# JiayuLi-997/IntEL-SIGIR2023

Hardware: AMD Instinct MI355X
Metric: train sessions/sec, IntEL fwd+IntBPRloss+bwd+Adam, synthetic Tmall-shape list=50 K=3, item / score tower 128 / 64 wide (higher is better)
Workload: dtype f32; 1 GPU; tmall: 1000000 items, list=50, K=3 rankers, I=30 intents, H=20, emb 64/64/64/64 (id/meta/score/ctx), BERT4Rec, 1 heads x 1 tied layers, f32, IntBPRloss loss, cal_diversity=0, uniform item ids, 8 resident batches; global_batch=4096, per_gpu_batch=4096, parallelism=dp1, table_adam=dense sweep over the whole table every step

## Files before the change

### intel_sigir2023_amd/csrc/attn_p3.hip

```cpp
#include "kernels.h"
#include "planes.h"
#include <stdlib.h>

namespace {

#define AP_QB 64
#define AP_KB 32
#define LOG2E_F 1.4426950408889634f
#ifndef AP_DKV_DUAL
#define AP_DKV_DUAL 0
#endif
#ifndef AP_DKV_PRE
#define AP_DKV_PRE 0
#endif
#ifndef AP_DKV_OCC
#define AP_DKV_OCC 3
#endif
#define LN2_F 0.6931471805599453f

typedef short ap_s16x4 __attribute__((ext_vector_type(4)));
typedef short ap_s16x8 __attribute__((ext_vector_type(8)));

template <int DKT>
struct P3Tile {
  static constexpr int RB = DKT * 32;
  static constexpr int NCH = DKT * 2;
  static constexpr int PLANE = AP_KB * RB;
  static constexpr int BYTES = 3 * PLANE;
  __device__ __forceinline__ static int swz(int row) {
    if (DKT == 8) return ((row & 3) << 1) | ((row >> 3) & 1) | ((((row >> 2) ^ (row >> 3)) & 1) << 3);
    const int u = (row >> 1) & 7;
    return ((u & 1) << 1) | ((u >> 2) & 1) | ((((u >> 1) ^ (u >> 2)) & 1) << 2);
  }
  __device__ __forceinline__ static int off(int row, int ch) { return RB * row + 16 * (ch ^ swz(row)); }
};

__device__ __forceinline__ void split8(const f32x4& a, const f32x4& b, bf16x8& h, bf16x8& m, bf16x8& l) {
#pragma unroll
  for (int i = 0; i < 4; ++i) {
    __bf16 hh, mm, ll;
    planes::split1(a[i], hh, mm, ll);
    h[i] = hh; m[i] = mm; l[i] = ll;
    planes::split1(b[i], hh, mm, ll);
    h[4 + i] = hh; m[4 + i] = mm; l[4 + i] = ll;
  }
}

template <int DKT>
struct P3Stage {
  static constexpr int NCH = DKT * 2, NCK = DKT / 4;
  f32x4 v[NCK][2];
  __device__ __forceinline__ void load(const float* __restrict__ base, int ldg, int coff, int r0, int nrow, int tid) {
#pragma unroll
    for (int n = 0; n < NCK; ++n) {
      const int i = tid + n * 256, r = i / NCH, ch = i - r * NCH, row = r0 + r;
      v[n][0] = v[n][1] = f32x4{0.f, 0.f, 0.f, 0.f};
      if (row < nrow) {
        const float* p = base + (size_t)row * ldg + coff + 8 * ch;
        v[n][0] = *reinterpret_cast<const f32x4*>(p);
        v[n][1] = *reinterpret_cast<const f32x4*>(p + 4);
      }
    }
  }
  __device__ __forceinline__ void store(unsigned char* tile, int tid) const {
    using TL = P3Tile<DKT>;
#pragma unroll
    for (int n = 0; n < NCK; ++n) {
      const int i = tid + n * 256, r = i / NCH, ch = i - r * NCH;
      bf16x8 h, m, l;
#if AP_ABLATE & 2
      for (int e = 0; e < 4; ++e) { h[e] = (__bf16)v[n][0][e]; h[4 + e] = (__bf16)v[n][1][e]; }
      m = h; l = h;
#else
      split8(v[n][0], v[n][1], h, m, l);
#endif
      unsigned char* d = tile + TL::off(r, ch);
      *reinterpret_cast<bf16x8*>(d) = h;
      *reinterpret_cast<bf16x8*>(d + TL::PLANE) = m;
      *reinterpret_cast<bf16x8*>(d + 2 * TL::PLANE) = l;
    }
  }
};

struct Frag3 { bf16x8 h, m, l; };
#define AP_MFMA(a, b, c) __builtin_amdgcn_mfma_f32_16x16x32_bf16(a, b, c, 0, 0, 0)
#ifndef AP_ABLATE
#define AP_ABLATE 0
#endif
__device__ __forceinline__ f32x4 ap_mma3(const bf16x8& ah, const bf16x8& am, const bf16x8& al, const bf16x8& bh, const bf16x8& bm, const bf16x8& bl, f32x4 c) {
#if AP_ABLATE & 1
  return AP_MFMA(ah, bh, c);
#else
  return planes::mma<3>(ah, am, al, bh, bm, bl, c);
#endif
}
__device__ __forceinline__ void mma3x2(const Frag3& a1, const Frag3& b1, f32x4& c1, const Frag3& a2, const Frag3& b2, f32x4& c2) {
#if AP_ABLATE & 1
  c1 = AP_MFMA(a1.h, b1.h, c1); c2 = AP_MFMA(a2.h, b2.h, c2);
  return;
#endif
  c1 = AP_MFMA(a1.m, b1.m, c1); c2 = AP_MFMA(a2.m, b2.m, c2);
  c1 = AP_MFMA(a1.h, b1.l, c1); c2 = AP_MFMA(a2.h, b2.l, c2);
  c1 = AP_MFMA(a1.l, b1.h, c1); c2 = AP_MFMA(a2.l, b2.h, c2);
  c1 = AP_MFMA(a1.h, b1.m, c1); c2 = AP_MFMA(a2.h, b2.m, c2);
  c1 = AP_MFMA(a1.m, b1.h, c1); c2 = AP_MFMA(a2.m, b2.h, c2);
  c1 = AP_MFMA(a1.h, b1.h, c1); c2 = AP_MFMA(a2.h, b2.h, c2);
}

template <int DKT>
__device__ __forceinline__ void own_row_planes(const float* __restrict__ rowp, bool ok, int g, Frag3 (&f)[DKT / 2]) {
#pragma unroll
  for (int c = 0; c < DKT / 2; ++c) {
    f32x4 a = f32x4{0.f, 0.f, 0.f, 0.f}, b = a;
    if (ok) {
      a = *reinterpret_cast<const f32x4*>(rowp + 32 * c + 8 * g);
      b = *reinterpret_cast<const f32x4*>(rowp + 32 * c + 8 * g + 4);
    }
    split8(a, b, f[c].h, f[c].m, f[c].l);
  }
}

template <int DKT>
__device__ __forceinline__ Frag3 row_frag(const unsigned char* tile, int roff, int t, int c) {
  using TL = P3Tile<DKT>;
  const unsigned char* p = tile + (roff ^ (64 * c)) + t * 16 * TL::RB;
  return Frag3{*reinterpret_cast<const bf16x8*>(p), *reinterpret_cast<const bf16x8*>(p + TL::PLANE), *reinterpret_cast<const bf16x8*>(p + 2 * TL::PLANE)};
}
template <int DKT, bool PRE = true>
__device__ __forceinline__ void row_mma2(const unsigned char* tile1, int t1, const Frag3 (&b1)[DKT / 2], f32x4& acc1, const unsigned char* tile2, int t2,
                                         const Frag3 (&b2)[DKT / 2], f32x4& acc2, int roff) {
  Frag3 a1 = row_frag<DKT>(tile1, roff, t1, 0), a2 = row_frag<DKT>(tile2, roff, t2, 0);
#pragma unroll
  for (int c = 0; c < DKT / 2; ++c) {
    Frag3 n1 = a1, n2 = a2;
    if (PRE && c + 1 < DKT / 2) {
      n1 = row_frag<DKT>(tile1, roff, t1, c + 1);
      n2 = row_frag<DKT>(tile2, roff, t2, c + 1);
    }
    mma3x2(a1, b1[c], acc1, a2, b2[c], acc2);
    if (!PRE && c + 1 < DKT / 2) {
      n1 = row_frag<DKT>(tile1, roff, t1, c + 1);
      n2 = row_frag<DKT>(tile2, roff, t2, c + 1);
    }
    a1 = n1; a2 = n2;
  }
}

__device__ __forceinline__ bf16x8 tr_frag(const unsigned char* plane, int off_lo, int off_hi) {
  const ap_s16x4 lo = __builtin_amdgcn_ds_read_tr16_b64_v4i16((__attribute__((address_space(3))) ap_s16x4*)(plane + off_lo));
  const ap_s16x4 hi = __builtin_amdgcn_ds_read_tr16_b64_v4i16((__attribute__((address_space(3))) ap_s16x4*)(plane + off_hi));
  return __builtin_bit_cast(bf16x8, __builtin_shufflevector(lo, hi, 0, 1, 2, 3, 4, 5, 6, 7));
}
template <int DKT>
__device__ __forceinline__ Frag3 tr_frag3(const unsigned char* tile, int tlo, int thi, int dt) {
  using TL = P3Tile<DKT>;
  const int lo = tlo ^ (32 * dt), hi = thi ^ (32 * dt);
  return Frag3{tr_frag(tile, lo, hi), tr_frag(tile + TL::PLANE, lo, hi), tr_frag(tile + 2 * TL::PLANE, lo, hi)};
}
template <int DKT, bool PRE = true>
__device__ __forceinline__ void tr_mma2(f32x4 (&acc1)[DKT], const unsigned char* tile1, const Frag3& b1, f32x4 (&acc2)[DKT], const unsigned char* tile2,
                                        const Frag3& b2, int tlo, int thi) {
  Frag3 a1 = tr_frag3<DKT>(tile1, tlo, thi, 0), a2 = tr_frag3<DKT>(tile2, tlo, thi, 0);
#pragma unroll
  for (int dt = 0; dt < DKT; ++dt) {
    Frag3 n1 = a1, n2 = a2;
    if (PRE && dt + 1 < DKT) {
      n1 = tr_frag3<DKT>(tile1, tlo, thi, dt + 1);
      n2 = tr_frag3<DKT>(tile2, tlo, thi, dt + 1);
    }
    mma3x2(a1, b1, acc1[dt], a2, b2, acc2[dt]);
    if (!PRE && dt + 1 < DKT) {
      n1 = tr_frag3<DKT>(tile1, tlo, thi, dt + 1);
      n2 = tr_frag3<DKT>(tile2, tlo, thi, dt + 1);
    }
    a1 = n1; a2 = n2;
  }
}
template <int DKT>
__device__ __forceinline__ f32x4 row_mma1(const unsigned char* tile, int t, const Frag3 (&b)[DKT / 2], f32x4 acc, int roff) {
#pragma unroll
  for (int c = 0; c < DKT / 2; ++c) {
    const Frag3 a = row_frag<DKT>(tile, roff, t, c);
    acc = ap_mma3(a.h, a.m, a.l, b[c].h, b[c].m, b[c].l, acc);
  }
  return acc;
}
template <int DKT>
__device__ __forceinline__ void tr_mma1(f32x4 (&acc)[DKT], const unsigned char* tile, const Frag3& b, int tlo, int thi) {
#pragma unroll
  for (int dt = 0; dt < DKT; ++dt) {
    const Frag3 a = tr_frag3<DKT>(tile, tlo, thi, dt);
    acc[dt] = ap_mma3(a.h, a.m, a.l, b.h, b.m, b.l, acc[dt]);
  }
}
template <int DKT>
__device__ __forceinline__ void tr_mma(f32x4 (&acc)[DKT], const unsigned char* tile, const Frag3& b, int tlo, int thi) {
  Frag3 a1 = tr_frag3<DKT>(tile, tlo, thi, 0), a2 = tr_frag3<DKT>(tile, tlo, thi, 1);
#pragma unroll
  for (int dt = 0; dt < DKT; dt += 2) {
    Frag3 n1 = a1, n2 = a2;
    if (dt + 2 < DKT) {
      n1 = tr_frag3<DKT>(tile, tlo, thi, dt + 2);
      n2 = tr_frag3<DKT>(tile, tlo, thi, dt + 3);
    }
    mma3x2(a1, b, acc[dt], a2, b, acc[dt + 1]);
    a1 = n1; a2 = n2;
  }
}
template <int DKT>
__device__ __forceinline__ void tr_addr(int lane, int& tlo, int& thi) {
  using TL = P3Tile<DKT>;
  const int p = lane & 15, g = lane >> 4, q = p >> 2, pp = p & 3;
  tlo = TL::off(4 * g + q, pp >> 1) + 8 * (pp & 1);
  thi = TL::off(16 + 4 * g + q, pp >> 1) + 8 * (pp & 1);
}

template <int DKT>
__device__ __forceinline__ void dim_store(float* __restrict__ rowp, const f32x4 (&acc)[DKT], int g, float mul) {
#pragma unroll
  for (int dt = 0; dt < DKT; ++dt) *reinterpret_cast<f32x4*>(rowp + 16 * dt + 4 * g) = acc[dt] * mul;
}

struct ApBlock { int bh, y; };
__device__ __forceinline__ ApBlock ap_block(int nbh, int ny) {
  const int id = blockIdx.x;
  if ((nbh & 7) == 0) {
    const int slot = id >> 3, g = slot / ny;
    return ApBlock{g * 8 + (id & 7), slot - g * ny};
  }
  const int bh = id / ny;
  return ApBlock{bh, id - bh * ny};
}

template <int DKT>
__global__ __launch_bounds__(256, DKT == 8 ? 2 : 3) void attn_fwd_p3_kernel(const float* __restrict__ qkv, int T, int d, int heads,
                                                                            const int* __restrict__ key_len, float scale, float* __restrict__ out,
                                                                            float* __restrict__ lse, const int* __restrict__ row_off) {
  using TL = P3Tile<DKT>;
  extern __shared__ __attribute__((aligned(16))) unsigned char smem_p3[];
  unsigned char* Ks = smem_p3;
  unsigned char* Vs = smem_p3 + TL::BYTES;
  const int tid = threadIdx.x, lane = tid & 63, wave = tid >> 6, p = lane & 15, g = lane >> 4;
  const int ny = (T + AP_QB - 1) / AP_QB;
  const ApBlock blk = ap_block((int)gridDim.x / ny, ny);
  const int b = blk.bh / heads, h = blk.bh - b * heads;
  const int dk = d / heads, ldg = 3 * d;
  const int nkeys = key_len ? min(key_len[b], T) : T;
  const int nrow = row_off ? nkeys : T;
  const size_t row0 = row_off ? (size_t)row_off[b] : (size_t)b * T;
  if (blk.y * AP_QB >= nrow) return;
  const float* base = qkv + row0 * ldg;
  const int q = blk.y * AP_QB + wave * 16 + p;
  Frag3 qf[DKT / 2];
  own_row_planes<DKT>(base + (size_t)q * ldg + h * dk, q < nrow, g, qf);
  f32x4 oT[DKT];
#pragma unroll
  for (int i = 0; i < DKT; ++i) oT[i] = f32x4{0.f, 0.f, 0.f, 0.f};
  float m_run = -INFINITY, l_run = 0.f;
  const int roff = TL::off(p, g);
  int tlo, thi;
  tr_addr<DKT>(lane, tlo, thi);
  const float scale2 = scale * LOG2E_F;

  P3Stage<DKT> kreg, vreg;
  kreg.load(base, ldg, d + h * dk, 0, nrow, tid);
  vreg.load(base, ldg, 2 * d + h * dk, 0, nrow, tid);
  for (int kb = 0; kb < nkeys; kb += AP_KB) {
    __syncthreads();
    kreg.store(Ks, tid);
    vreg.store(Vs, tid);
    __syncthreads();
    if (kb + AP_KB < nkeys) {
      kreg.load(base, ldg, d + h * dk, kb + AP_KB, nrow, tid);
      vreg.load(base, ldg, 2 * d + h * dk, kb + AP_KB, nrow, tid);
    }
// ... 140 lines not shown
  }
}

template <int DKT>
__global__ __launch_bounds__(256, 4) void attn_bwd_dq_ds_p3_kernel(const float* __restrict__ qkv, const float* __restrict__ dS, int ldS, int T, int d,
                                                                   int heads, const int* __restrict__ key_len, float* __restrict__ dqkv,
                                                                   const int* __restrict__ row_off) {
  extern __shared__ __attribute__((aligned(16))) unsigned char smem_p3[];
  unsigned char* Ks = smem_p3;
  const int tid = threadIdx.x, lane = tid & 63, wave = tid >> 6, p = lane & 15, g = lane >> 4;
  const int ny = (T + AP_QB - 1) / AP_QB;
  const ApBlock blk = ap_block((int)gridDim.x / ny, ny);
  const int b = blk.bh / heads, h = blk.bh - b * heads;
  const int dk = d / heads, ldg = 3 * d;
  const int nkeys = key_len ? min(key_len[b], T) : T;
  const int nrow = row_off ? nkeys : T;
  const size_t row0 = row_off ? (size_t)row_off[b] : (size_t)b * T;
  if (blk.y * AP_QB >= nrow) return;
  const float* base = qkv + row0 * ldg;
  const int q = blk.y * AP_QB + wave * 16 + p;
  const bool qok = q < nrow;
  const float* dSq = dS + ((size_t)blk.bh * T + (qok ? q : 0)) * ldS;
  f32x4 dqT[DKT];
#pragma unroll
  for (int i = 0; i < DKT; ++i) dqT[i] = f32x4{0.f, 0.f, 0.f, 0.f};
  int tlo, thi;
  tr_addr<DKT>(lane, tlo, thi);
  P3Stage<DKT> kreg;
  kreg.load(base, ldg, d + h * dk, 0, nrow, tid);
  for (int kb = 0; kb < nkeys; kb += AP_KB) {
    __syncthreads();
    kreg.store(Ks, tid);
    __syncthreads();
    if (kb + AP_KB < nkeys) kreg.load(base, ldg, d + h * dk, kb + AP_KB, nrow, tid);
    if (blk.y * AP_QB + wave * 16 >= nrow) continue;
    f32x4 dsT[2];
#pragma unroll
    for (int kt = 0; kt < 2; ++kt) {
      const int key0 = kb + kt * 16 + 4 * g;
      dsT[kt] = f32x4{0.f, 0.f, 0.f, 0.f};
      if (qok && key0 < ldS && key0 < nkeys) dsT[kt] = *reinterpret_cast<const f32x4*>(dSq + key0);
#pragma unroll
      for (int r = 0; r < 4; ++r) dsT[kt][r] = key0 + r < nkeys ? dsT[kt][r] : 0.f;
    }
    Frag3 df;
    split8(dsT[0], dsT[1], df.h, df.m, df.l);
    tr_mma<DKT>(dqT, Ks, df, tlo, thi);
  }
  if (qok) dim_store<DKT>(dqkv + (row0 + q) * ldg + h * dk, dqT, g, 1.f);
}

}

bool attn_p3_supported(int T, int dk) {
  static const int on = [] { const char* e = getenv("INTEL_ATTN_P3"); return (e && e[0] == '0') ? 0 : 1; }();
  return on && gemm_planes() == 3 && T > 64 && (dk == 64 || dk == 128);
}

#define AP_DISPATCH(DKT_RT, CALL) \
  if ((DKT_RT) == 4) { constexpr int DKT = 4; CALL; } else { constexpr int DKT = 8; CALL; }

int launch_attn_p3_fwd(const float* qkv, int B, int T, int d, int heads, const int* key_len, float* out, float* lse, hipStream_t st, const int* row_off) {
  const int dk = d / heads, dkt = dk / 16;
  INTEL_CHECK_ARG(dk == 64 || dk == 128, "attention (bf16-plane kernels): head dim %d", dk);
  const float scale = 1.0f / sqrtf((float)dk);
  dim3 grid(B * heads * cdiv(T, AP_QB));
  AP_DISPATCH(dkt, {
    size_t smem = (size_t)2 * P3Tile<DKT>::BYTES;
    allow_lds(attn_fwd_p3_kernel<DKT>, smem);
    LAUNCH_S(B * heads, T, dk, 4.0 * B * T * (double)T * d, 16.0 * B * T * (double)d, attn_fwd_p3_kernel<DKT>, grid, dim3(256), smem, st, qkv, T, d, heads, key_len, scale, out, lse, row_off);
  });
  INTEL_CHECK_LAUNCH();
  return 0;
}

int launch_attn_p3_bwd(const float* qkv, const float* dout, const float* lse, const float* dsum, int B, int T, int d, int heads, const int* key_len,
                       float* dqkv, float* dS, int ldS, hipStream_t st, const int* row_off) {
  const int dk = d / heads, dkt = dk / 16;
  INTEL_CHECK_ARG(dk == 64 || dk == 128, "attention (bf16-plane kernels): head dim %d", dk);
  const float scale = 1.0f / sqrtf((float)dk);
  dim3 grid(B * heads * cdiv(T, AP_QB));
  AP_DISPATCH(dkt, {
    size_t smem = (size_t)2 * P3Tile<DKT>::BYTES + 2 * AP_KB * sizeof(float);
    allow_lds(attn_bwd_dkv_p3_kernel<DKT>, smem);
    LAUNCH_S(B * heads, T, dk, 8.0 * B * T * (double)T * d, 24.0 * B * T * (double)d, attn_bwd_dkv_p3_kernel<DKT>, grid, dim3(256), smem, st, qkv, dout, lse, dsum, T, d, heads,
             key_len, scale, dqkv, dS, ldS, row_off);
  });
  INTEL_CHECK_LAUNCH();
  AP_DISPATCH(dkt, {
    size_t smem = (size_t)P3Tile<DKT>::BYTES;
    allow_lds(attn_bwd_dq_ds_p3_kernel<DKT>, smem);
    LAUNCH_S(B * heads, T, dk, 2.0 * B * T * (double)T * d, 8.0 * B * T * (double)d + 4.0 * B * heads * (double)T * T, attn_bwd_dq_ds_p3_kernel<DKT>, grid, dim3(256), smem, st, qkv, dS,
             ldS, T, d, heads, key_len, dqkv, row_off);
  });
  INTEL_CHECK_LAUNCH();
  return 0;
}
```

### intel_sigir2023_amd/csrc/attn_seq.hip

```cpp
#include <stdio.h>
#include <stdlib.h>
#include "kernels.h"

namespace {

__device__ __forceinline__ int perm16(int r) { return (r & ~15) | ((r & 3) << 2) | ((r >> 2) & 3); }
__device__ __forceinline__ float gmax16(float v) {
  v = fmaxf(v, __shfl_xor(v, 16));
  return fmaxf(v, __shfl_xor(v, 32));
}
__device__ __forceinline__ float gsum16(float v) {
  v += __shfl_xor(v, 16);
  return v + __shfl_xor(v, 32);
}

typedef short s16x4 __attribute__((ext_vector_type(4)));
typedef __bf16 bf16x4s __attribute__((ext_vector_type(4)));
template <bool BF>
__device__ __forceinline__ f32x4 mma4(const f32x4& a, const f32x4& b, f32x4 c) {
  if (BF) {
    const bf16x4s ab = bf16x4s{(__bf16)a[0], (__bf16)a[1], (__bf16)a[2], (__bf16)a[3]};
    const bf16x4s bb = bf16x4s{(__bf16)b[0], (__bf16)b[1], (__bf16)b[2], (__bf16)b[3]};
    return __builtin_amdgcn_mfma_f32_16x16x16bf16_1k(__builtin_bit_cast(s16x4, ab), __builtin_bit_cast(s16x4, bb), c, 0, 0, 0);
  }
#pragma unroll
  for (int s = 0; s < 4; ++s) c = mfma16(a[s], b[s], c);
  return c;
}

template <bool H>
__device__ __forceinline__ f32x4 ldx4(const float* __restrict__ base, size_t off) {
  if (H) {
    const bf16x4s v = *reinterpret_cast<const bf16x4s*>(reinterpret_cast<const __bf16*>(base) + off);
    return f32x4{(float)v[0], (float)v[1], (float)v[2], (float)v[3]};
  }
  return *reinterpret_cast<const f32x4*>(base + off);
}
template <bool H>
__device__ __forceinline__ void stx4(float* __restrict__ base, size_t off, const f32x4& v) {
  if (H) *reinterpret_cast<bf16x4s*>(reinterpret_cast<__bf16*>(base) + off) = bf16x4s{(__bf16)v[0], (__bf16)v[1], (__bf16)v[2], (__bf16)v[3]};
  else *reinterpret_cast<f32x4*>(base + off) = v;
}

template <int DKT, int NT>
struct SeqP {
  static constexpr int DK = DKT * 16;
  static constexpr int PW = 4 / NT;
  static constexpr int TP = NT * 16;
  static constexpr int ROWS = PW * TP;
  static constexpr int CPR = DKT * 4;
  static constexpr int BUF = ROWS * DK;
  static constexpr int IPW = ROWS * CPR / 256;
};

template <int DKT, int NT, bool PERM>
// ... 226 lines not shown
};

template <int DKT, int NT, bool PERM>
__device__ __forceinline__ bool seq_src(int i, int bh0, int BH, int T, int heads, int& rl, int& c4, size_t& grow, int& hcol,
                                        const int* __restrict__ row_off = nullptr, const int* __restrict__ key_len = nullptr) {
  using C = SeqCfg<DKT, NT>;
  rl = i / C::C4;
  c4 = i - rl * C::C4;
  const int sl = rl / C::TP, r = rl - sl * C::TP;
  const int rho = PERM ? perm16(r) : r;
  const int bh = bh0 + sl;
  int b = bh, h = 0;
  if (heads > 1) { b = bh / heads; h = bh - b * heads; }
  hcol = h * C::DK + c4 * 4;
  if (row_off) {
    if (bh >= BH) { grow = 0; return false; }
    grow = (size_t)row_off[b] + rho;
    return rho < min(key_len[b], T);
  }
  grow = (size_t)b * T + rho;
  return bh < BH && rho < T;
}

template <int DKT, int NT, bool PERM, bool TWO>
__device__ __forceinline__ void stage_seq2(float* dst0, const float* __restrict__ src0, int ld0, int coff0, float* dst1,
                                           const float* __restrict__ src1, int ld1, int coff1, int bh0, int BH, int T,
                                           int heads, int tid) {
  using C = SeqCfg<DKT, NT>;
  f32x4 v0[C::ITERS], v1[C::ITERS];
#pragma unroll
  for (int it = 0; it < C::ITERS; ++it) {
    int rl, c4, hcol;
    size_t grow;
    const bool ok = seq_src<DKT, NT, PERM>(tid + it * 256, bh0, BH, T, heads, rl, c4, grow, hcol);
    const size_t gr = ok ? grow : 0;
    const int hc = ok ? hcol : 0;
    const f32x4 zero = f32x4{0.f, 0.f, 0.f, 0.f};
    const f32x4 t0 = *reinterpret_cast<const f32x4*>(src0 + gr * ld0 + coff0 + hc);
    v0[it] = ok ? t0 : zero;
    if (TWO) {
      const f32x4 t1 = *reinterpret_cast<const f32x4*>(src1 + gr * ld1 + coff1 + hc);
      v1[it] = ok ? t1 : zero;
    }
  }
#pragma unroll
  for (int it = 0; it < C::ITERS; ++it) {
    const int i = tid + it * 256;
    const int rl = i / C::C4, c4 = i - rl * C::C4;
    *reinterpret_cast<f32x4*>(dst0 + rl * C::LD + c4 * 4) = v0[it];
    if (TWO) *reinterpret_cast<f32x4*>(dst1 + rl * C::LD + c4 * 4) = v1[it];
  }
}

template <int DKT, int NT, int LS, bool BF = false, bool H16 = false>
__global__ __launch_bounds__(256, 2) void attn_seq_bwd_fused_kernel(const float* __restrict__ qkv, const float* __restrict__ out,
                                                              const float* __restrict__ dout, const float* __restrict__ lse,
                                                              int BH, int T, int d, int heads, const int* __restrict__ key_len,
                                                              const int* __restrict__ row_off, float c2, float scale,
                                                              float* __restrict__ dqkv) {
  using C = SeqCfg<DKT, NT>;
  constexpr int LD = C::LD, DK = C::DK, DQ = DKT / 4, TP = C::TP, NSTEPS = (NT - 1) * 4 + LS;
  extern __shared__ __attribute__((aligned(16))) float smem[];
  float* Qs = smem;
  float* Os = smem + C::ROWS * LD;
  float* Ls = smem + C::ROWS * LD + C::OSZ;
  float* Ds = Ls + C::ROWS;
  const int tid = threadIdx.x, lane = tid & 63, wave = tid >> 6, j = lane >> 4, p = lane & 15;
  const int bh0 = blockIdx.x * C::PW, ldg = 3 * d;
  const int slot = wave / NT, tile = wave - slot * NT, bh = bh0 + slot;
  const bool live = slot < C::PW && bh < BH;
  int b = live ? bh : 0, h = 0;
  if (heads > 1) { b = (live ? bh : 0) / heads; h = (live ? bh : 0) - b * heads; }
  const int key = tile * 16 + p;
  const size_t base = row_off ? (size_t)row_off[b] : (size_t)b * T;
  const int tb = row_off ? min(key_len[b], T) : T;
  const bool kok = live && key < tb;
  f32x4 kf[DKT], vf[DKT];
#pragma unroll
  for (int g = 0; g < DKT; ++g) {
    const int col = g * 16 + 4 * j;
    const bool ok = kok && col < DK;
    const size_t off = ok ? (base + key) * ldg + d + h * DK + col : 0;
    const f32x4 tk = ldx4<H16>(qkv, off), tv = ldx4<H16>(qkv, off + (ok ? d : 0));
    kf[g] = ok ? tk : f32x4{0.f, 0.f, 0.f, 0.f};
    vf[g] = ok ? tv : f32x4{0.f, 0.f, 0.f, 0.f};
  }
  {
    f32x4 vq[C::ITERS], vo[C::ITERS];
#pragma unroll
    for (int it = 0; it < C::ITERS; ++it) {
      int rl, c4, hcol;
      size_t grow;
      const bool ok = seq_src<DKT, NT, true>(tid + it * 256, bh0, BH, T, heads, rl, c4, grow, hcol, row_off, key_len);
      const size_t gr = ok ? grow : 0;
      const int hc = ok ? hcol : 0;
      const f32x4 zero = f32x4{0.f, 0.f, 0.f, 0.f};
      const f32x4 tq = ldx4<H16>(qkv, gr * ldg + hc);
      const f32x4 to = ldx4<H16>(dout, gr * d + hc);
      vq[it] = ok ? tq : zero;
      vo[it] = ok ? to : zero;
    }
#pragma unroll
    for (int it = 0; it < C::ITERS; ++it) {
      const int i = tid + it * 256;
      const int rl = i / C::C4, c4 = i - rl * C::C4;
      *reinterpret_cast<f32x4*>(Qs + rl * LD + c4 * 4) = vq[it];
      *reinterpret_cast<f32x4*>(Os + rl * LD + c4 * 4) = vo[it];
    }
    if (tid < C::ROWS) {
      const int sl = tid / TP, r = tid - sl * TP, rho = perm16(r), bb = bh0 + sl;
      const int tbb = (row_off && bb < BH) ? min(key_len[heads > 1 ? bb / heads : bb], T) : T;
      Ls[tid] = (bb < BH && rho < tbb) ? -1.44269504088896340736f * lse[(size_t)bb * T + rho] : -INFINITY;
// ... 210 lines not shown
bool attn_seq_supported(int T, int dk) {
  static const int off = [] { const char* e = getenv("INTEL_ATTN_SEQ"); return (e && e[0] == '0') ? 1 : 0; }();
  return !off && T >= 1 && T <= 64 && (dk == 64 || dk == 128);
}

int launch_attn_seq_fwd(const float* qkv, int B, int T, int d, int heads, const int* key_len, float* out, float* lse,
                        hipStream_t st, const int* row_off) {
  INTEL_CHECK_ARG(!row_off || key_len, "attn_seq: packed rows need the session lengths");
  const int dk = d / heads, dkt = dk / 16, BH = B * heads;
  const int nt = cdiv(T, 16), ls = cdiv(T - (nt - 1) * 16, 4);
  const float scale = 1.0f / sqrtf((float)dk);
  SEQ_DISPATCH3(dkt, nt, ls, {
    using C = SeqP<DKT, NT>;
    const size_t smem = (size_t)4 * C::BUF * sizeof(float);
    const int per_cu = (int)((size_t)160 * 1024 / smem);
    const int grid = min(cdiv(BH, C::PW), num_cus() * (per_cu < 1 ? 1 : per_cu));
    if (gemm_planes() == 1) {
      allow_lds((attn_seq_fwd_kernel<DKT, NT, LS, true>), smem);
      LAUNCH_S(BH, T, dk, 4.0 * B * T * (double)T * d, 16.0 * B * T * (double)d, (attn_seq_fwd_kernel<DKT, NT, LS, true>), dim3(grid), dim3(256), smem, st, qkv, BH, T, d, heads, key_len, row_off, scale * 1.44269504088896340736f, scale, out, lse);
    } else {
      allow_lds((attn_seq_fwd_kernel<DKT, NT, LS>), smem);
      LAUNCH_S(BH, T, dk, 4.0 * B * T * (double)T * d, 16.0 * B * T * (double)d, (attn_seq_fwd_kernel<DKT, NT, LS>), dim3(grid), dim3(256), smem, st, qkv, BH, T, d, heads, key_len, row_off, scale * 1.44269504088896340736f, scale, out, lse);
    }
  });
  INTEL_CHECK_LAUNCH();
  return 0;
}

size_t attn_seq_bwd_scratch_floats(int B, int T, int heads) {
  const size_t tp = (size_t)cdiv(T, 16) * 16;
  return (size_t)B * heads * tp * tp;
}

bool attn_seq_packed_supported(int T, int dk) {
  return attn_seq_supported(T, dk);
}

bool attn_seq_h16_supported(int T, int dk) { return attn_seq_packed_supported(T, dk) && gemm_planes() == 1; }

int launch_attn_seq_bwd(const float* qkv, const float* out, const float* dout, const float* lse, int B, int T, int d,
                        int heads, const int* key_len, float* dqkv, float* dS, hipStream_t st, const int* row_off, int h16) {
  INTEL_CHECK_ARG(!h16 || attn_seq_h16_supported(T, d / heads), "attn_seq: bf16-stored q/k/v need the fused backward in bf16 mode");
  INTEL_CHECK_ARG(!row_off || (key_len && attn_seq_packed_supported(T, d / heads)), "attn_seq: packed rows need the fused backward and the session lengths");
  const int dk = d / heads, dkt = dk / 16, BH = B * heads;
  const int nt = cdiv(T, 16), ls = cdiv(T - (nt - 1) * 16, 4);
  const float scale = 1.0f / sqrtf((float)dk);
  {
    SEQ_DISPATCH3(dkt, nt, ls, {
      using C = SeqCfg<DKT, NT>;
      const size_t smem = (size_t)(C::ROWS * C::LD + C::OSZ + (1 + NT) * C::ROWS) * sizeof(float);
      if (h16) {
        allow_lds((attn_seq_bwd_fused_kernel<DKT, NT, LS, true, true>), smem);
        LAUNCH_S(BH, T, dk, 10.0 * B * T * (double)T * d, 16.0 * B * T * (double)d, (attn_seq_bwd_fused_kernel<DKT, NT, LS, true, true>), dim3(cdiv(BH, C::PW)), dim3(256), smem, st, qkv, out, dout, lse, BH, T, d, heads, key_len, row_off, scale * 1.44269504088896340736f, scale, dqkv);
      } else if (gemm_planes() == 1) {
        allow_lds((attn_seq_bwd_fused_kernel<DKT, NT, LS, true>), smem);
        LAUNCH_S(BH, T, dk, 10.0 * B * T * (double)T * d, 24.0 * B * T * (double)d, (attn_seq_bwd_fused_kernel<DKT, NT, LS, true>), dim3(cdiv(BH, C::PW)), dim3(256), smem, st, qkv, out, dout, lse, BH, T, d, heads, key_len, row_off, scale * 1.44269504088896340736f, scale, dqkv);
      } else {
        allow_lds((attn_seq_bwd_fused_kernel<DKT, NT, LS>), smem);
        LAUNCH_S(BH, T, dk, 10.0 * B * T * (double)T * d, 24.0 * B * T * (double)d, (attn_seq_bwd_fused_kernel<DKT, NT, LS>), dim3(cdiv(BH, C::PW)), dim3(256), smem, st, qkv, out, dout, lse, BH, T, d, heads, key_len, row_off, scale * 1.44269504088896340736f, scale, dqkv);
      }
    });
    INTEL_CHECK_LAUNCH();
    return 0;
  }
}
```

### intel_sigir2023_amd/csrc/kernels.h

```cpp
#pragma once
#include "common.h"

static inline size_t packed_floats(int Kd, int Nd) { return (size_t)rup(Kd, 16) * rup(Nd, 16); }
int launch_pack_b(const float* W, int ldw, int Kd, int Nd, int trans, float* P, int nt_off, hipStream_t st,
                  int g_off = 0, int KG_total = 0);

void pack_batch_begin();
int pack_batch_end(hipStream_t st);

struct GemmEpilogue {
  const float* bias = nullptr;
  int relu = 0;
  const float* mask = nullptr;
  int ldmask = 0;
  const float* res = nullptr;
  int ldres = 0;
  const float* gamma = nullptr;
  const float* beta = nullptr;
  float* xhat = nullptr;
  int ldxhat = 0;
  float* rstd = nullptr;
  int accumulate = 0;
  int no_out = 0;
  const void* b3 = nullptr;
  int a_bf16 = 0;
  int c_bf16 = 0;
  int mask_bf16 = 0;
};
void gemm_set_planes(int planes);
int gemm_planes();
size_t packed_b3_bytes(int Kd, int Nd);
int launch_pack_b3(const float* Pf32, int Kd, int Nd, void* Pb3, hipStream_t st);
int pack_b3_flush(hipStream_t st);
int launch_vec_copy(const float* src, float* dst, int n, hipStream_t st);
int vec_copy_flush(hipStream_t st);
void pack_jobs_reset();
int launch_gemm_rows(const float* A, int lda, int M, int K, const float* Bp, int N, float* C, int ldc,
                     const GemmEpilogue& ep, hipStream_t st);
size_t wgrad_slab_floats(int M, int N, int K);

struct ReduceQueue;
ReduceQueue* redq_create();
void redq_destroy(ReduceQueue* q);
void redq_reset(ReduceQueue* q, float* arena, size_t arena_floats);
float* redq_alloc(ReduceQueue* q, size_t floats);
void redq_push(ReduceQueue* q, const float* slabs, size_t stride, int S, int rows, int cols, float* out, int ldo,
               int accumulate);
int redq_flush(ReduceQueue* q, hipStream_t st);
void redq_set_tag(ReduceQueue* q, int tag);
int redq_flush_tag(ReduceQueue* q, int tag, hipStream_t st);

struct WgradSplit { int n; float* dW[4]; float* db[4]; int acc[4]; int dy_bf16 = 0; };
int launch_wgrad(const float* dY, int lddy, const float* X, int ldx, int M, int N, int K, float* dW, int lddw,
                 float* db, int accumulate, float* slabs, hipStream_t st, ReduceQueue* q = nullptr, const WgradSplit* split = nullptr,
                 int io16 = 0);

bool smallk_supported(int N, int K);
int launch_linear_smallk(const float* X, int ldx, int M, int K, const float* W, const float* bias, int N, float* Y, int ldy,
                         int relu, hipStream_t st, const float* pos = nullptr, const int* row_t = nullptr);
int smallk_wgrad_slabs(int M);
void wgrad_batch_begin();
int wgrad_batch_flush(hipStream_t st);
void wgrad_batch_reset();
int launch_wgrad_smallk(const float* dY, int lddy, const float* X, int ldx, int M, int N, int K, float* dW, int lddw, float* db,
                        int accumulate, float* slabs, hipStream_t st, ReduceQueue* q = nullptr);

bool attn_seq_packed_supported(int T, int dk);
bool attn_packed_supported(int T, int dk);
int launch_attn_fwd(const float* qkv, int B, int T, int d, int heads, const int* key_len, float* out, float* lse,
                    hipStream_t st, const int* row_off = nullptr);
bool attn_p3_supported(int T, int dk);
int launch_attn_p3_fwd(const float* qkv, int B, int T, int d, int heads, const int* key_len, float* out, float* lse, hipStream_t st, const int* row_off);
int launch_attn_p3_bwd(const float* qkv, const float* dout, const float* lse, const float* dsum, int B, int T, int d, int heads, const int* key_len,
                       float* dqkv, float* dS, int ldS, hipStream_t st, const int* row_off);
bool attn_seq_supported(int T, int dk);
int launch_attn_seq_fwd(const float* qkv, int B, int T, int d, int heads, const int* key_len, float* out, float* lse,
                        hipStream_t st, const int* row_off = nullptr);
size_t attn_seq_bwd_scratch_floats(int B, int T, int heads);
bool attn_seq_h16_supported(int T, int dk);
int launch_attn_seq_bwd(const float* qkv, const float* out, const float* dout, const float* lse, int B, int T, int d,
                        int heads, const int* key_len, float* dqkv, float* dS, hipStream_t st, const int* row_off = nullptr, int h16 = 0);
size_t attn_bwd_scratch_floats(int B, int T, int d, int heads);
int launch_attn_bwd(const float* qkv, const float* out, const float* dout, const float* lse, int B, int T, int d,
                    int heads, const int* key_len, float* dqkv, float* scratch, hipStream_t st, const int* row_off = nullptr, int h16 = 0);

bool tower_fused_supported(int L, int d, int heads);
bool tower_fused_wanted(int train, int d);
struct TowerInput {
  const float* tab0 = nullptr; const int* idx0 = nullptr; int d0 = 0;
  const float* tab1 = nullptr; const int* idx1 = nullptr;
};
int launch_tower_fwd_fused(const float* X, int B, int L, int d, int heads, const void* Wqkv_b3, const void* W1_b3, const void* W2_b3,
                           const float* b1, const float* b2, const float* gamma, const float* beta, float* out, int train,
                           float* QKV, float* A, float* LSE, float* R1, float* XH, float* RSTD, hipStream_t st, int qkv16 = 0, const TowerInput* in = nullptr);

bool tower_bwd_fused_supported(int L, int d, int heads);
bool tower_bwd_fused_wanted(int d);
size_t tower_bwd_slab_floats(int B, int d);
int tower_bwd_fused_scope(int d);
int launch_tower_bwd_fused(const float* X, const float* A, const float* LSE, const float* dZ, int B, int L, int d, int heads, const void* Wqkv_b3,
                           const void* W1_b3, const void* W2T_b3, const void* W1T_b3, const void* WqkvT_b3, const float* b1, float* dQKV, float* dX,
                           float* const* grads, const int* accumulate, ReduceQueue* q, hipStream_t st, int a16 = 0, int dqkv16 = 0);

bool linear_bwd_pair_supported(int M, int d);
size_t linear_bwd_pair_slab_floats(int M, int d);
int launch_linear_bwd_pair(const float* dY, int lddy, const float* X, int ldx, int M, int d, const void* WT_b3, int relu_mask, float* dXout, int ldo,
                           float* dW, float* db, int acc_w, int acc_b, ReduceQueue* q, hipStream_t st);

bool linear_bwd_qkv_supported(int M, int d, int nb);
size_t linear_bwd_qkv_slab_floats(int M, int d, int nb);
int launch_linear_bwd_qkv(const float* dY, int lddy, const float* X, int ldx, const float* res, int ldr, int M, int d, int nb, const void* WT_b3, float* dXout, int ldo,
                          float* const* dW, float* const* db, const int* acc, ReduceQueue* q, hipStream_t st);

bool tower32_supported(int L, int d, int heads, int layers, int train);
size_t tower32_slab_floats(int B);
struct Tower32Dropout { float p; unsigned long long seed; unsigned stream0; const float* ext; };
int launch_tower32_fwd(const float* X, int B, int L, int heads, int layers, const float* Wq, const float* Wk, const float* Wv, const float* W1,
                       const float* b1, const float* W2, const float* b2, const float* gamma, const float* beta, float* out, hipStream_t st,
                       const Tower32Dropout* drop = nullptr);
int launch_tower32_bwd(const float* X, const float* dout, int B, int L, int heads, int layers, const float* Wq, const float* Wk, const float* Wv,
                       const float* W1, const float* b1, const float* W2, const float* b2, const float* gamma, const float* beta, float* dX,
                       float* const* grads, const int* accumulate, ReduceQueue* q, hipStream_t st, const Tower32Dropout* drop = nullptr, int share8 = 8);

// ... 38 lines not shown
```

Baseline: 1.272 million sessions/s.

## Add 3-plane bf16 MFMA path for short-sequence fused attention backward

Moves the shared 3-plane bf16 split helpers (tile layout, split8, fragment loaders) into a common header. Adds a new path for the short-sequence fused attention backward (dk=64) that splits Q, dO, K and V into hi/mid/lo bf16 planes and computes P, dP, dV, dK and dQ with bf16 MFMA triple products, replacing the existing f32 path. It uses 512 threads split into two wave roles, and reuses the dead dO LDS region to park dS rows for the dQ pass. It is enabled whenever gemm planes is 3 and INTEL_ATTN_P3 is not 0, which trades extra LDS, extra split work and more synchronisation for matrix-core throughput.

New measurement: 1.262 million sessions/s, median of 3. Within noise of the previous version (-0.8%).

```diff
diff --git a/intel_sigir2023_amd/csrc/attn_p3.hip b/intel_sigir2023_amd/csrc/attn_p3.hip
--- a/intel_sigir2023_amd/csrc/attn_p3.hip
+++ b/intel_sigir2023_amd/csrc/attn_p3.hip
@@ -1,5 +1,5 @@
 #include "kernels.h"
-#include "planes.h"
+#include "attn_planes.h"
 #include <stdlib.h>
 
 namespace {
@@ -18,33 +18,7 @@
 #endif
 #define LN2_F 0.6931471805599453f
 
-typedef short ap_s16x4 __attribute__((ext_vector_type(4)));
-typedef short ap_s16x8 __attribute__((ext_vector_type(8)));
-
-template <int DKT>
-struct P3Tile {
-  static constexpr int RB = DKT * 32;
-  static constexpr int NCH = DKT * 2;
-  static constexpr int PLANE = AP_KB * RB;
-  static constexpr int BYTES = 3 * PLANE;
-  __device__ __forceinline__ static int swz(int row) {
-    if (DKT == 8) return ((row & 3) << 1) | ((row >> 3) & 1) | ((((row >> 2) ^ (row >> 3)) & 1) << 3);
-    const int u = (row >> 1) & 7;
-    return ((u & 1) << 1) | ((u >> 2) & 1) | ((((u >> 1) ^ (u >> 2)) & 1) << 2);
-  }
-  __device__ __forceinline__ static int off(int row, int ch) { return RB * row + 16 * (ch ^ swz(row)); }
-};
-
-__device__ __forceinline__ void split8(const f32x4& a, const f32x4& b, bf16x8& h, bf16x8& m, bf16x8& l) {
-#pragma unroll
-  for (int i = 0; i < 4; ++i) {
-    __bf16 hh, mm, ll;
-    planes::split1(a[i], hh, mm, ll);
-    h[i] = hh; m[i] = mm; l[i] = ll;
-    planes::split1(b[i], hh, mm, ll);
-    h[4 + i] = hh; m[4 + i] = mm; l[4 + i] = ll;
-  }
-}
+using namespace ap3;
 
 template <int DKT>
 struct P3Stage {
@@ -82,7 +56,6 @@
   }
 };
 
-struct Frag3 { bf16x8 h, m, l; };
 #define AP_MFMA(a, b, c) __builtin_amdgcn_mfma_f32_16x16x32_bf16(a, b, c, 0, 0, 0)
 #ifndef AP_ABLATE
 #define AP_ABLATE 0
@@ -107,25 +80,6 @@
   c1 = AP_MFMA(a1.h, b1.h, c1); c2 = AP_MFMA(a2.h, b2.h, c2);
 }
 
-template <int DKT>
-__device__ __forceinline__ void own_row_planes(const float* __restrict__ rowp, bool ok, int g, Frag3 (&f)[DKT / 2]) {
-#pragma unroll
-  for (int c = 0; c < DKT / 2; ++c) {
-    f32x4 a = f32x4{0.f, 0.f, 0.f, 0.f}, b = a;
-    if (ok) {
-      a = *reinterpret_cast<const f32x4*>(rowp + 32 * c + 8 * g);
-      b = *reinterpret_cast<const f32x4*>(rowp + 32 * c + 8 * g + 4);
-    }
-    split8(a, b, f[c].h, f[c].m, f[c].l);
-  }
-}
-
-template <int DKT>
-__device__ __forceinline__ Frag3 row_frag(const unsigned char* tile, int roff, int t, int c) {
-  using TL = P3Tile<DKT>;
-  const unsigned char* p = tile + (roff ^ (64 * c)) + t * 16 * TL::RB;
-  return Frag3{*reinterpret_cast<const bf16x8*>(p), *reinterpret_cast<const bf16x8*>(p + TL::PLANE), *reinterpret_cast<const bf16x8*>(p + 2 * TL::PLANE)};
-}
 template <int DKT, bool PRE = true>
 __device__ __forceinline__ void row_mma2(const unsigned char* tile1, int t1, const Frag3 (&b1)[DKT / 2], f32x4& acc1, const unsigned char* tile2, int t2,
                                          const Frag3 (&b2)[DKT / 2], f32x4& acc2, int roff) {
@@ -146,17 +100,6 @@
   }
 }
 
-__device__ __forceinline__ bf16x8 tr_frag(const unsigned char* plane, int off_lo, int off_hi) {
-  const ap_s16x4 lo = __builtin_amdgcn_ds_read_tr16_b64_v4i16((__attribute__((address_space(3))) ap_s16x4*)(plane + off_lo));
-  const ap_s16x4 hi = __builtin_amdgcn_ds_read_tr16_b64_v4i16((__attribute__((address_space(3))) ap_s16x4*)(plane + off_hi));
-  return __builtin_bit_cast(bf16x8, __builtin_shufflevector(lo, hi, 0, 1, 2, 3, 4, 5, 6, 7));
-}
-template <int DKT>
-__device__ __forceinline__ Frag3 tr_frag3(const unsigned char* tile, int tlo, int thi, int dt) {
-  using TL = P3Tile<DKT>;
-  const int lo = tlo ^ (32 * dt), hi = thi ^ (32 * dt);
-  return Frag3{tr_frag(tile, lo, hi), tr_frag(tile + TL::PLANE, lo, hi), tr_frag(tile + 2 * TL::PLANE, lo, hi)};
-}
 template <int DKT, bool PRE = true>
 __device__ __forceinline__ void tr_mma2(f32x4 (&acc1)[DKT], const unsigned char* tile1, const Frag3& b1, f32x4 (&acc2)[DKT], const unsigned char* tile2,
                                         const Frag3& b2, int tlo, int thi) {
@@ -207,20 +150,6 @@
     a1 = n1; a2 = n2;
   }
 }
-template <int DKT>
-__device__ __forceinline__ void tr_addr(int lane, int& tlo, int& thi) {
-  using TL = P3Tile<DKT>;
-  const int p = lane & 15, g = lane >> 4, q = p >> 2, pp = p & 3;
-  tlo = TL::off(4 * g + q, pp >> 1) + 8 * (pp & 1);
-  thi = TL::off(16 + 4 * g + q, pp >> 1) + 8 * (pp & 1);
-}
-
-template <int DKT>
-__device__ __forceinline__ void dim_store(float* __restrict__ rowp, const f32x4 (&acc)[DKT], int g, float mul) {
-#pragma unroll
-  for (int dt = 0; dt < DKT; ++dt) *reinterpret_cast<f32x4*>(rowp + 16 * dt + 4 * g) = acc[dt] * mul;
-}
-
 struct ApBlock { int bh, y; };
 __device__ __forceinline__ ApBlock ap_block(int nbh, int ny) {
   const int id = blockIdx.x;
@@ -467,10 +396,11 @@
 
 }
 
-bool attn_p3_supported(int T, int dk) {
+bool attn_p3_enabled() {
   static const int on = [] { const char* e = getenv("INTEL_ATTN_P3"); return (e && e[0] == '0') ? 0 : 1; }();
-  return on && gemm_planes() == 3 && T > 64 && (dk == 64 || dk == 128);
-}
+  return on && gemm_planes() == 3;
+}
+bool attn_p3_supported(int T, int dk) { return attn_p3_enabled() && T > 64 && (dk == 64 || dk == 128); }
 
 #define AP_DISPATCH(DKT_RT, CALL) \
   if ((DKT_RT) == 4) { constexpr int DKT = 4; CALL; } else { constexpr int DKT = 8; CALL; }
diff --git a/intel_sigir2023_amd/csrc/attn_planes.h b/intel_sigir2023_amd/csrc/attn_planes.h
--- /dev/null
+++ b/intel_sigir2023_amd/csrc/attn_planes.h
@@ -0,0 +1,80 @@
+#pragma once
+#include "planes.h"
+
+namespace ap3 {
+
+typedef short ap_s16x4 __attribute__((ext_vector_type(4)));
+
+template <int DKT, int R = 32>
+struct P3Tile {
+  static constexpr int RB = DKT * 32;
+  static constexpr int NCH = DKT * 2;
+  static constexpr int PLANE = R * RB;
+  static constexpr int BYTES = 3 * PLANE;
+  __device__ __forceinline__ static int swz(int row) {
+    if (DKT == 8) return ((row & 3) << 1) | ((row >> 3) & 1) | ((((row >> 2) ^ (row >> 3)) & 1) << 3);
+    const int u = (row >> 1) & 7;
+    return ((u & 1) << 1) | ((u >> 2) & 1) | ((((u >> 1) ^ (u >> 2)) & 1) << 2);
+  }
+  __device__ __forceinline__ static int off(int row, int ch) { return RB * row + 16 * (ch ^ swz(row)); }
+};
+
+__device__ __forceinline__ void split8(const f32x4& a, const f32x4& b, bf16x8& h, bf16x8& m, bf16x8& l) {
+#pragma unroll
+  for (int i = 0; i < 4; ++i) {
+    __bf16 hh, mm, ll;
+    planes::split1(a[i], hh, mm, ll);
+    h[i] = hh; m[i] = mm; l[i] = ll;
+    planes::split1(b[i], hh, mm, ll);
+    h[4 + i] = hh; m[4 + i] = mm; l[4 + i] = ll;
+  }
+}
+
+struct Frag3 { bf16x8 h, m, l; };
+
+template <int DKT>
+__device__ __forceinline__ void own_row_planes(const float* __restrict__ rowp, bool ok, int g, Frag3 (&f)[DKT / 2]) {
+#pragma unroll
+  for (int c = 0; c < DKT / 2; ++c) {
+    f32x4 a = f32x4{0.f, 0.f, 0.f, 0.f}, b = a;
+    if (ok) {
+      a = *reinterpret_cast<const f32x4*>(rowp + 32 * c + 8 * g);
+      b = *reinterpret_cast<const f32x4*>(rowp + 32 * c + 8 * g + 4);
+    }
+    split8(a, b, f[c].h, f[c].m, f[c].l);
+  }
+}
+
+template <int DKT, int R = 32>
+__device__ __forceinline__ Frag3 row_frag(const unsigned char* tile, int roff, int t, int c) {
+  using TL = P3Tile<DKT, R>;
+  const unsigned char* p = tile + (roff ^ (64 * c)) + t * 16 * TL::RB;
+  return Frag3{*reinterpret_cast<const bf16x8*>(p), *reinterpret_cast<const bf16x8*>(p + TL::PLANE), *reinterpret_cast<const bf16x8*>(p + 2 * TL::PLANE)};
+}
+
+__device__ __forceinline__ bf16x8 tr_frag(const unsigned char* plane, int off_lo, int off_hi) {
+  const ap_s16x4 lo = __builtin_amdgcn_ds_read_tr16_b64_v4i16((__attribute__((address_space(3))) ap_s16x4*)(plane + off_lo));
+  const ap_s16x4 hi = __builtin_amdgcn_ds_read_tr16_b64_v4i16((__attribute__((address_space(3))) ap_s16x4*)(plane + off_hi));
+  return __builtin_bit_cast(bf16x8, __builtin_shufflevector(lo, hi, 0, 1, 2, 3, 4, 5, 6, 7));
+}
+template <int DKT, int R = 32>
+__device__ __forceinline__ Frag3 tr_frag3(const unsigned char* tile, int tlo, int thi, int dt) {
+  using TL = P3Tile<DKT, R>;
+  const int lo = tlo ^ (32 * dt), hi = thi ^ (32 * dt);
+  return Frag3{tr_frag(tile, lo, hi), tr_frag(tile + TL::PLANE, lo, hi), tr_frag(tile + 2 * TL::PLANE, lo, hi)};
+}
+template <int DKT>
+__device__ __forceinline__ void tr_addr(int lane, int& tlo, int& thi) {
+  using TL = P3Tile<DKT>;
+  const int p = lane & 15, g = lane >> 4, q = p >> 2, pp = p & 3;
+  tlo = TL::off(4 * g + q, pp >> 1) + 8 * (pp & 1);
+  thi = TL::off(16 + 4 * g + q, pp >> 1) + 8 * (pp & 1);
+}
+
+template <int DKT>
+__device__ __forceinline__ void dim_store(float* __restrict__ rowp, const f32x4 (&acc)[DKT], int g, float mul) {
+#pragma unroll
+  for (int dt = 0; dt < DKT; ++dt) *reinterpret_cast<f32x4*>(rowp + 16 * dt + 4 * g) = acc[dt] * mul;
+}
+
+}
diff --git a/intel_sigir2023_amd/csrc/attn_seq.hip b/intel_sigir2023_amd/csrc/attn_seq.hip
--- a/intel_sigir2023_amd/csrc/attn_seq.hip
+++ b/intel_sigir2023_amd/csrc/attn_seq.hip
@@ -1,6 +1,7 @@
 #include <stdio.h>
 #include <stdlib.h>
 #include "kernels.h"
+#include "attn_planes.h"
 
 namespace {
 
@@ -333,12 +334,214 @@
   }
 }
 
-template <int DKT, int NT, int LS, bool BF = false, bool H16 = false>
-__global__ __launch_bounds__(256, 2) void attn_seq_bwd_fused_kernel(const float* __restrict__ qkv, const float* __restrict__ out,
+template <int DKT, int NT>
+struct SeqP3 {
+  static constexpr int DK = DKT * 16;
+  static constexpr int NB = NT <= 2 ? 1 : 2;
+  static constexpr int TP = 32 * NB;
+  static constexpr int PW = 2 / NB;
+  static constexpr int ROWS = 64;
+  static constexpr int NKT = 2 * NB;
+  static constexpr int TPD = TP + 8;
+  using TL = ap3::P3Tile<DKT, ROWS>;
+  static constexpr int LDS = 2 * TL::BYTES + (1 + NKT) * ROWS * (int)sizeof(float);
+  static_assert(ROWS * TPD * (int)sizeof(float) <= TL::BYTES, "the parked dS rows fit the dead dO image");
+};
+
+template <int DKT, int R>
+__device__ __forceinline__ f32x4 p3_row(const unsigned char* tile, int roff, int t, const ap3::Frag3 (&b)[DKT / 2], f32x4 acc) {
+#pragma unroll
+  for (int c = 0; c < DKT / 2; ++c) {
+    const ap3::Frag3 a = ap3::row_frag<DKT, R>(tile, roff, t, c);
+    acc = planes::mma<3>(a.h, a.m, a.l, b[c].h, b[c].m, b[c].l, acc);
+  }
+  return acc;
+}
+template <int DKT, int R, int N, int D0>
+__device__ __forceinline__ void p3_tr(f32x4 (&acc)[N], const unsigned char* block, const ap3::Frag3& b, int tlo, int thi) {
+#pragma unroll
+  for (int i = 0; i < N; ++i) {
+    const ap3::Frag3 a = ap3::tr_frag3<DKT, R>(block, tlo, thi, D0 + i);
+    acc[i] = planes::mma<3>(a.h, a.m, a.l, b.h, b.m, b.l, acc[i]);
+  }
+}
+
+template <int DKT, int NT>
+__device__ __forceinline__ void attn_seq_bwd_p3(const float* __restrict__ qkv, const float* __restrict__ dout, const float* __restrict__ lse, int BH,
+                                                int T, int d, int heads, const int* __restrict__ key_len, const int* __restrict__ row_off, float c2,
+                                                float scale, float* __restrict__ dqkv, unsigned char* smem) {
+  using C = SeqP3<DKT, NT>;
+  using TL = typename C::TL;
+  constexpr int DK = C::DK, TP = C::TP, NB = C::NB, NKT = C::NKT, ROWS = C::ROWS, HD = DKT / 2;
+  unsigned char* Qs = smem;
+  unsigned char* Os = smem + TL::BYTES;
+  float* Ls = reinterpret_cast<float*>(smem + 2 * TL::BYTES);
+  float* Ds = Ls + ROWS;
+  const int tid = threadIdx.x, lane = tid & 63, p = lane & 15, g = lane >> 4;
+  const int wave = __builtin_amdgcn_readfirstlane(tid >> 6);
+  const int role = wave >> 2, tw = wave & 3;
+  const int slot = tw / NKT, tile = tw - slot * NKT;
+  const int bh0 = blockIdx.x * C::PW, ldg = 3 * d, bh = bh0 + slot;
+  const bool live = bh < BH;
+  int b, h;
+  split_pair(live ? bh : 0, heads, b, h);
+  const size_t base = row_off ? (size_t)row_off[b] : (size_t)b * T;
+  const int tb = row_off ? min(key_len[b], T) : T;
+  const int nkeys = live ? (key_len ? min(key_len[b], T) : T) : 0;
+  const int key = tile * 16 + p;
+  const bool kok = live && key < tb;
+  const bool key_live = key < nkeys;
+  ap3::Frag3 kf[HD], vf[HD];
+  {
+    constexpr int NCH = TL::NCH, NCK = ROWS * NCH / 512;
+    f32x4 vq[NCK][2], vo[NCK][2];
+#pragma unroll
+    for (int n = 0; n < NCK; ++n) {
+      const int i = tid + n * 512, r = i / NCH, ch = i - r * NCH;
+      const int sl = r / TP, rho = r - sl * TP, bb = bh0 + sl;
+      int sb, sh;
+      split_pair(bb < BH ? bb : 0, heads, sb, sh);
+      const bool ok = bb < BH && rho < (row_off ? min(key_len[sb], T) : T);
+      const size_t grow = (row_off ? (size_t)row_off[sb] : (size_t)sb * T) + rho;
+      vq[n][0] = vq[n][1] = vo[n][0] = vo[n][1] = f32x4{0.f, 0.f, 0.f, 0.f};
+      if (ok) {
+        const float* qp = qkv + grow * ldg + sh * DK + 8 * ch;
+        const float* op = dout + grow * d + sh * DK + 8 * ch;
+        vq[n][0] = *reinterpret_cast<const f32x4*>(qp);
+        vq[n][1] = *reinterpret_cast<const f32x4*>(qp + 4);
+        vo[n][0] = *reinterpret_cast<const f32x4*>(op);
+        vo[n][1] = *reinterpret_cast<const f32x4*>(op + 4);
+      }
+    }
+    const float* krow = qkv + (base + (kok ? key : 0)) * ldg + d + h * DK;
+    ap3::own_row_planes<DKT>(krow, kok, g, kf);
+    if (role) ap3::own_row_planes<DKT>(krow + d, kok, g, vf);
+    if (tid < ROWS) {
+      const int sl = tid / TP, rho = tid - sl * TP, bb = bh0 + sl;
+      const int tbb = (row_off && bb < BH) ? min(key_len[heads > 1 ? bb / heads : bb], T) : T;
+      Ls[tid] = (bb < BH && rho < tbb) ? -1.44269504088896340736f * lse[(size_t)bb * T + rho] : -INFINITY;
+    }
+#pragma unroll
+    for (int n = 0; n < NCK; ++n) {
+      const int i = tid + n * 512, r = i / NCH, ch = i - r * NCH;
+      bf16x8 hq, mq, lq, ho, mo, lo;
+      ap3::split8(vq[n][0], vq[n][1], hq, mq, lq);
+      ap3::split8(vo[n][0], vo[n][1], ho, mo, lo);
+      const int o = TL::off(r, ch);
+      *reinterpret_cast<bf16x8*>(Qs + o) = hq;
+      *reinterpret_cast<bf16x8*>(Qs + o + TL::PLANE) = mq;
+      *reinterpret_cast<bf16x8*>(Qs + o + 2 * TL::PLANE) = lq;
+      *reinterpret_cast<bf16x8*>(Os + o) = ho;
+      *reinterpret_cast<bf16x8*>(Os + o + TL::PLANE) = mo;
+      *reinterpret_cast<bf16x8*>(Os + o + 2 * TL::PLANE) = lo;
+    }
+  }
+  __syncthreads();
+  const int roff = TL::off(p, g);
+  int tlo, thi;
+  ap3::tr_addr<DKT>(lane, tlo, thi);
+  const unsigned char* Qp = Qs + slot * TP * TL::RB;
+  const unsigned char* Op = Os + slot * TP * TL::RB;
+  const float* Lp = Ls + slot * TP;
+  float* Dp = Ds + slot * TP * NKT;
+  f32x4 prs[NKT], dsk[NKT];
+  f32x4 acc[DKT];
+#pragma unroll
+  for (int i = 0; i < DKT; ++i) acc[i] = f32x4{0.f, 0.f, 0.f, 0.f};
+  if (live) {
+#pragma unroll
+    for (int qt = 0; qt < NKT; ++qt) {
+      const f32x4 sa = p3_row<DKT, ROWS>(Qp, roff, qt, kf, f32x4{0.f, 0.f, 0.f, 0.f});
+      f32x4 dp = f32x4{0.f, 0.f, 0.f, 0.f};
+      if (role) dp = p3_row<DKT, ROWS>(Op, roff, qt, vf, dp);
+#pragma unroll
+      for (int r = 0; r < 4; ++r) {
+        const int ql = qt * 16 + 4 * g + r;
+        const float pv = key_live ? __builtin_amdgcn_exp2f(__builtin_fmaf(sa[r], c2, Lp[ql])) : 0.f;
+        prs[qt][r] = pv;
+        if (role) {
+          const float x = planes::row16_sum(pv * dp[r]);
+          if (p == 0) Dp[ql * NKT + tile] = x;
+        }
+      }
+      dsk[qt] = dp;
+      if (!role && (qt & 1)) {
+        ap3::Frag3 pf;
+        ap3::split8(prs[qt - 1], prs[qt], pf.h, pf.m, pf.l);
+        p3_tr<DKT, ROWS, DKT, 0>(acc, Op + (qt - 1) * 16 * TL::RB, pf, tlo, thi);
+      }
+    }
+  }
+  __syncthreads();
+  if (live) {
+    if (role) {
+#pragma unroll
+      for (int qt = 0; qt < NKT; ++qt) {
+#pragma unroll
+        for (int r = 0; r < 4; ++r) {
+          const int ql = qt * 16 + 4 * g + r;
+          float delta = 0.f;
+#pragma unroll
+          for (int t = 0; t < NKT; ++t) delta += Dp[ql * NKT + t];
+          dsk[qt][r] = prs[qt][r] * (dsk[qt][r] - delta) * scale;
+        }
+        if (qt & 1) {
+          ap3::Frag3 df;
+          ap3::split8(dsk[qt - 1], dsk[qt], df.h, df.m, df.l);
+          p3_tr<DKT, ROWS, DKT, 0>(acc, Qp + (qt - 1) * 16 * TL::RB, df, tlo, thi);
+        }
+      }
+    }
+    if (kok) ap3::dim_store<DKT>(dqkv + (base + key) * ldg + h * DK + (role ? d : 2 * d), acc, g, 1.f);
+  }
+  __syncthreads();
+  unsigned char* Ks = Qs;
+  float* Dsh = reinterpret_cast<float*>(Os);
+  if (live) {
+    if (!role) {
+#pragma unroll
+      for (int c = 0; c < HD; ++c) {
+        unsigned char* dst = Ks + TL::off(slot * TP + key, 4 * c + g);
+        *reinterpret_cast<bf16x8*>(dst) = kf[c].h;
+        *reinterpret_cast<bf16x8*>(dst + TL::PLANE) = kf[c].m;
+        *reinterpret_cast<bf16x8*>(dst + 2 * TL::PLANE) = kf[c].l;
+      }
+    } else {
+#pragma unroll
+      for (int qt = 0; qt < NKT; ++qt)
+#pragma unroll
+        for (int r = 0; r < 4; ++r) Dsh[(slot * TP + qt * 16 + 4 * g + r) * C::TPD + key] = dsk[qt][r];
+    }
+  }
+  __syncthreads();
+  if (!live) return;
+  const int q = tile * 16 + p;
+  const float* Dq = Dsh + (slot * TP + q) * C::TPD;
+  f32x4 dqT[HD];
+#pragma unroll
+  for (int i = 0; i < HD; ++i) dqT[i] = f32x4{0.f, 0.f, 0.f, 0.f};
+#pragma unroll
+  for (int kb = 0; kb < NB; ++kb) {
+    ap3::Frag3 df;
+    ap3::split8(*reinterpret_cast<const f32x4*>(Dq + 32 * kb + 4 * g), *reinterpret_cast<const f32x4*>(Dq + 32 * kb + 16 + 4 * g), df.h, df.m, df.l);
+    const unsigned char* blk = Ks + (slot * TP + 32 * kb) * TL::RB;
+    if (role) p3_tr<DKT, ROWS, HD, HD>(dqT, blk, df, tlo, thi);
+    else p3_tr<DKT, ROWS, HD, 0>(dqT, blk, df, tlo, thi);
+  }
+  if (q < tb) ap3::dim_store<HD>(dqkv + (base + q) * ldg + h * DK + role * HD * 16, dqT, g, 1.f);
+}
+
+template <int DKT, int NT, int LS, bool BF = false, bool H16 = false, bool P3 = false>
+__global__ __launch_bounds__(P3 ? 512 : 256, P3 && DKT == 4 ? 4 : 2) void attn_seq_bwd_fused_kernel(const float* __restrict__ qkv, const float* __restrict__ out,
                                                               const float* __restrict__ dout, const float* __restrict__ lse,
                                                               int BH, int T, int d, int heads, const int* __restrict__ key_len,
                                                               const int* __restrict__ row_off, float c2, float scale,
                                                               float* __restrict__ dqkv) {
+  if constexpr (P3) {
+    extern __shared__ __attribute__((aligned(16))) unsigned char smem_seq_p3[];
+    attn_seq_bwd_p3<DKT, NT>(qkv, dout, lse, BH, T, d, heads, key_len, row_off, c2, scale, dqkv, smem_seq_p3);
+    return;
+  }
   using C = SeqCfg<DKT, NT>;
   constexpr int LD = C::LD, DK = C::DK, DQ = DKT / 4, TP = C::TP, NSTEPS = (NT - 1) * 4 + LS;
   extern __shared__ __attribute__((aligned(16))) float smem[];
@@ -655,6 +858,11 @@
       if (h16) {
         allow_lds((attn_seq_bwd_fused_kernel<DKT, NT, LS, true, true>), smem);
         LAUNCH_S(BH, T, dk, 10.0 * B * T * (double)T * d, 16.0 * B * T * (double)d, (attn_seq_bwd_fused_kernel<DKT, NT, LS, true, true>), dim3(cdiv(BH, C::PW)), dim3(256), smem, st, qkv, out, dout, lse, BH, T, d, heads, key_len, row_off, scale * 1.44269504088896340736f, scale, dqkv);
+      } else if (attn_p3_enabled() && DKT == 4) {
+        constexpr int NTP = NT <= 2 ? 2 : 4;
+        const size_t smem3 = (size_t)SeqP3<DKT, NTP>::LDS;
+        allow_lds((attn_seq_bwd_fused_kernel<DKT, NTP, 4, false, false, true>), smem3);
+        LAUNCH_S(BH, T, dk, 10.0 * B * T * (double)T * d, 24.0 * B * T * (double)d, (attn_seq_bwd_fused_kernel<DKT, NTP, 4, false, false, true>), dim3(cdiv(BH, SeqP3<DKT, NTP>::PW)), dim3(512), smem3, st, qkv, out, dout, lse, BH, T, d, heads, key_len, row_off, scale * 1.44269504088896340736f, scale, dqkv);
       } else if (gemm_planes() == 1) {
         allow_lds((attn_seq_bwd_fused_kernel<DKT, NT, LS, true>), smem);
         LAUNCH_S(BH, T, dk, 10.0 * B * T * (double)T * d, 24.0 * B * T * (double)d, (attn_seq_bwd_fused_kernel<DKT, NT, LS, true>), dim3(cdiv(BH, C::PW)), dim3(256), smem, st, qkv, out, dout, lse, BH, T, d, heads, key_len, row_off, scale * 1.44269504088896340736f, scale, dqkv);
diff --git a/intel_sigir2023_amd/csrc/kernels.h b/intel_sigir2023_amd/csrc/kernels.h
--- a/intel_sigir2023_amd/csrc/kernels.h
+++ b/intel_sigir2023_amd/csrc/kernels.h
@@ -69,6 +69,7 @@
 bool attn_packed_supported(int T, int dk);
 int launch_attn_fwd(const float* qkv, int B, int T, int d, int heads, const int* key_len, float* out, float* lse,
                     hipStream_t st, const int* row_off = nullptr);
+bool attn_p3_enabled();
 bool attn_p3_supported(int T, int dk);
 int launch_attn_p3_fwd(const float* qkv, int B, int T, int d, int heads, const int* key_len, float* out, float* lse, hipStream_t st, const int* row_off);
 int launch_attn_p3_bwd(const float* qkv, const float* dout, const float* lse, const float* dsum, int B, int T, int d, int heads, const int* key_len,
```
